# Okrio/tinyrecurrentunet

Measured on AMD Instinct MI355X. Metric: 16 kHz frames/sec (train step), higher is better.
Workload: dtype f32; 1 GPU; config/tiny.json TRU-Net (C_in=4 incl. PCEN), 64 x 4 s 16 kHz pairs per GPU, n_fft 512 hop 128, full fp32 train step; mfma=fp32 forward, bf16x3 backward, fp32_mfma=bf16x3-bwd, frames_per_gpu=32064, global_batch=64, parallelism=dp1

## Files before the change

tinyrecurrentunet_amd/csrc/dma_common.hpp:

```cpp
#pragma once
#include "common.hpp"

namespace {

typedef __attribute__((address_space(3))) void* lds_ptr_t;

#define VMCNT_0_31_(W_)                                                                                                \
    W_(0) W_(1) W_(2) W_(3) W_(4) W_(5) W_(6) W_(7) W_(8) W_(9) W_(10) W_(11) W_(12) W_(13) W_(14) W_(15)             \
    W_(16) W_(17) W_(18) W_(19) W_(20) W_(21) W_(22) W_(23) W_(24) W_(25) W_(26) W_(27) W_(28) W_(29) W_(30) W_(31)
#define VMCNT_32_60_(W_)                                                                                               \
    W_(32) W_(33) W_(34) W_(35) W_(36) W_(37) W_(38) W_(39) W_(40) W_(41) W_(42) W_(43) W_(44) W_(45) W_(46) W_(47)   \
    W_(48) W_(49) W_(50) W_(51) W_(52) W_(53) W_(54) W_(55) W_(56) W_(57) W_(58) W_(59) W_(60)
#define VMCNT_CASE_(k) case k: asm volatile("s_waitcnt vmcnt(" #k ")" ::: "memory"); break;
template <int MAXN>
__device__ __forceinline__ void wait_vmcnt_exact(int n) {
    static_assert(MAXN == 31 || MAXN == 60, "ranges with a case list");
    if constexpr (MAXN == 31) {
        switch (n) {
            VMCNT_0_31_(VMCNT_CASE_)
            default: asm volatile("s_waitcnt vmcnt(0)" ::: "memory"); break;
        }
    } else {
        switch (n) {
            VMCNT_0_31_(VMCNT_CASE_) VMCNT_32_60_(VMCNT_CASE_)
            default: asm volatile("s_waitcnt vmcnt(0)" ::: "memory"); break;
        }
    }
}
#undef VMCNT_CASE_
#undef VMCNT_32_60_
#undef VMCNT_0_31_

__device__ __forceinline__ int swz_off(int r, int pc) { return r * 32 + 4 * (pc ^ ((r >> 1) & 7)); }

__device__ __forceinline__ __amdgpu_buffer_rsrc_t buffer_rsrc(const void* base) {
    return __builtin_amdgcn_make_buffer_rsrc(const_cast<void*>(base), 0, 0x7fffffff, 0x00020000);
}

__device__ __forceinline__ int wave_uniform(int v) { return __builtin_amdgcn_readfirstlane(v); }

}
```

tinyrecurrentunet_amd/csrc/gemm_common.hpp:

```cpp
#pragma once
#include "dma_common.hpp"

namespace {


constexpr int NT = TRUNET_TILE_FRAMES;

template <int CT>
struct BVec;
template <>
struct BVec<4> { typedef f32x4 type; };
template <>
struct BVec<2> { typedef f32x2 type; };
template <>
struct BVec<1> { typedef float type; };

template <int CT>
__device__ __forceinline__ float vget(const typename BVec<CT>::type& v, int i) {
    if constexpr (CT == 1) return v; else return v[i];
}
template <int CT>
__device__ __forceinline__ void vset(typename BVec<CT>::type& v, int i, float x) {
    if constexpr (CT == 1) v = x; else v[i] = x;
}

struct SegPos { bool valid; int q; };

__device__ __forceinline__ SegPos seg_pos(const trunet_seg& sg, int p) {
    int qn = p * sg.pos_mul + sg.pos_off;
    SegPos r;
    const int sh = sg.pos_div >> 1;
    r.q = qn >> sh;
    r.valid = (qn >= 0) && ((qn & sh) == 0) && (r.q < sg.L);
    return r;
}

struct ChunkIt {
    int tile, tile_end, p, n0, s, cc, ach, cbase;
    bool valid;
    bool placed;
};

template <int KC, int FT = NT>
__device__ __forceinline__ void it_enter_tile(const trunet_gemm_args& a, ChunkIt& it) {
    it.valid = it.tile < it.tile_end;
    if (!it.valid) return;
    if (!it.placed) {
        const int nt = it.tile / a.P;
        it.p = a.p_begin + (it.tile - nt * a.P);
        it.n0 = nt * FT;
        it.placed = true;
    }
    it.s = 0; it.cc = 0; it.ach = 0; it.cbase = 0;
#ifdef GEMM_SIMPLE_IT
    return;
#endif
    while (it.s < a.nseg - 1 && !seg_pos(a.seg[it.s], it.p).valid) {
        it.ach += (a.seg[it.s].nchan + KC - 1) / KC;
        it.cbase += a.seg[it.s].nchan;
        ++it.s;
    }
}

template <int KC, int FT = NT>
__device__ __forceinline__ bool it_next(const trunet_gemm_args& a, ChunkIt& it) {
#ifdef GEMM_SIMPLE_IT
    if (++it.cc < (a.seg[0].nchan + KC - 1) / KC) return false;
    it.cc = 0;
    ++it.tile;
    if (++it.p == a.p_begin + a.P) { it.p = a.p_begin; it.n0 += FT; }
    it.valid = it.tile < it.tile_end;
    return true;
#endif
    const int nck = (a.seg[it.s].nchan + KC - 1) / KC;
    if (++it.cc < nck) return false;
    it.ach += nck;
    it.cbase += a.seg[it.s].nchan;
    it.cc = 0;
    ++it.s;
    while (it.s < a.nseg && !seg_pos(a.seg[it.s], it.p).valid) {
        it.ach += (a.seg[it.s].nchan + KC - 1) / KC;
        it.cbase += a.seg[it.s].nchan;
        ++it.s;
    }
    if (it.s < a.nseg) return false;
    ++it.tile;
    if (++it.p == a.p_begin + a.P) { it.p = a.p_begin; it.n0 += FT; }
    it_enter_tile<KC, FT>(a, it);
    return true;
}

__device__ __forceinline__ void wait_vmcnt(int n) {
    switch (n >> 2) {
        case 0: asm volatile("s_waitcnt vmcnt(0)" ::: "memory"); break;
        case 1: asm volatile("s_waitcnt vmcnt(4)" ::: "memory"); break;
        case 2: asm volatile("s_waitcnt vmcnt(8)" ::: "memory"); break;
        case 3: asm volatile("s_waitcnt vmcnt(12)" ::: "memory"); break;
        case 4: asm volatile("s_waitcnt vmcnt(16)" ::: "memory"); break;
        case 5: asm volatile("s_waitcnt vmcnt(20)" ::: "memory"); break;
        case 6: asm volatile("s_waitcnt vmcnt(24)" ::: "memory"); break;
        case 7: asm volatile("s_waitcnt vmcnt(28)" ::: "memory"); break;
        case 8: asm volatile("s_waitcnt vmcnt(32)" ::: "memory"); break;
        case 9: asm volatile("s_waitcnt vmcnt(36)" ::: "memory"); break;
        case 10: asm volatile("s_waitcnt vmcnt(40)" ::: "memory"); break;
        case 11: asm volatile("s_waitcnt vmcnt(44)" ::: "memory"); break;
        default: asm volatile("s_waitcnt vmcnt(48)" ::: "memory"); break;
    }
}

}
```

tinyrecurrentunet_amd/csrc/gemm_conv.hip:

```cpp
#include <cstdlib>
#include "common.hpp"

#include "gemm_common.hpp"

namespace {


template <int RS, int KC, bool TWO, int EPL, int NW>
__global__ __launch_bounds__(64 * NW, (EPL == 0 || NW == 8) ? 2 : 1) void conv_gemm_kernel(const trunet_gemm_args a, const int NB) {
    constexpr int FT = 32 * NW;
    constexpr int CT = RS;
    constexpr int CG = 4 / RS;
    constexpr int MB = 32 * RS;
    constexpr int KP = KC / 2;
    constexpr int NSRC = TWO ? 2 : 1;
    constexpr int CHF = KC * FT * NSRC;
    constexpr int LPW = (KC / 8) * NSRC;
    typedef typename BVec<CT>::type bvec;
    extern __shared__ __attribute__((aligned(16))) float smem[];

    const int tid = threadIdx.x;
    const int lane = tid & 63;
    const int wave8 = __builtin_amdgcn_readfirstlane(tid >> 6);
    const int half = wave8 >> 2;
    const int wave = wave8 & 3;
    const int rs = wave % RS;
    const int cg = wave / RS;
    const int h = lane >> 5;
    const int c = lane & 31;
    const int mblk = blockIdx.y;

    int nck_total = 0, nchan_total = 0;
    for (int s = 0; s < a.nseg; ++s) {
        nck_total += (a.seg[s].nchan + KC - 1) / KC;
        nchan_total += a.seg[s].nchan;
    }
    float* A_lds = smem;
    float* R_lds = A_lds + (size_t)nck_total * RS * (KP * 64);
    f32x4* C_lds = (f32x4*)(R_lds + (size_t)NB * CHF);
    float* E_lds = (float*)(C_lds + nchan_total);

    const int ntn = a.NP / FT;
    const int total_tiles = a.P * ntn;
    ChunkIt cur;
    cur.placed = false;
    cur.tile = (int)(((long long)blockIdx.x * total_tiles) / gridDim.x);
    cur.tile_end = (int)(((long long)(blockIdx.x + 1) * total_tiles) / gridDim.x);
    const bool has_work = cur.tile < cur.tile_end;

    float st1[16], st2[16];
#pragma unroll
    for (int r = 0; r < 16; ++r) { st1[r] = 0.f; st2[r] = 0.f; }

    if (has_work) {
        const int totalA = nck_total * RS * (KP * 64);
        for (int idx = tid; idx < totalA; idx += 64 * NW) {
            const int j = idx & 3;
            const int ln = (idx >> 2) & 63;
            const int rest = idx >> 8;
            const int kg = rest % (KP / 4);
            const int rest2 = rest / (KP / 4);
            const int rr = rest2 % RS;
            const int ch = rest2 / RS;
            int s = 0, cc = ch;
            while (cc >= (a.seg[s].nchan + KC - 1) / KC) { cc -= (a.seg[s].nchan + KC - 1) / KC; ++s; }
            const int kk = 4 * kg + j;
            const int ci = cc * KC + 2 * kk + (ln >> 5);
            const int m = mblk * MB + 32 * rr + (ln & 31);
            const bool ok = ci < a.seg[s].nchan && m < a.M;
            const float v = a.W[(size_t)(min(m, a.M - 1) + a.w_m_off) * a.ldw_m +
                                (size_t)min(ci, a.seg[s].nchan - 1) * a.ldw_c + a.seg[s].woff];
            A_lds[idx] = ok ? v : 0.f;
        }
        int base = 0;
        for (int s = 0; s < a.nseg; ++s) {
            const trunet_seg& sg = a.seg[s];
            for (int ci = tid; ci < sg.nchan; ci += 64 * NW) {
                f32x4 k;
                if (TWO) {
                    const bool on = sg.mode == TRUNET_PRO_BNBWD;
                    k[0] = on ? sg.c0[ci] : 1.f; k[1] = on ? sg.c1[ci] : 0.f; k[2] = on ? sg.c2[ci] : 0.f; k[3] = 0.f;
                } else {
                    const bool on = sg.mode == TRUNET_PRO_BNRELU;
                    k[0] = on ? sg.c0[ci] : 1.f; k[1] = on ? sg.c1[ci] : 0.f; k[2] = on ? 0.f : -3.0e38f; k[3] = 0.f;
                }
                C_lds[base + ci] = k;
            }
            base += sg.nchan;
        }
        for (int r = tid; r < MB; r += 64 * NW) {
            const int m = mblk * MB + r;
            const int mg = m + a.m_out_off;
            const bool ok = m < a.M;
            E_lds[r] = (ok && (a.epi & TRUNET_EPI_BIAS)) ? a.bias[mg] : 0.f;
            E_lds[MB + r] = (ok && EPL > 0) ? a.e0[mg] : 0.f;
            E_lds[2 * MB + r] = (ok && EPL > 0) ? a.e1[mg] : 0.f;
            E_lds[3 * MB + r] = (ok && EPL > 0 && a.e2) ? a.e2[mg] : 0.f;
        }
    }
    __syncthreads();

    if (has_work) {
        auto issue_dma = [&](const ChunkIt& it, int slot) {
            const trunet_seg& sg = a.seg[it.s];
            const int q = seg_pos(sg, it.p).q;
            float* dst = R_lds + (size_t)slot * CHF;
            const size_t boff = (size_t)q * a.NP + it.n0;
            const unsigned rstride = (unsigned)sg.L * (unsigned)a.NP;
            const float* b0 = sg.src0 + boff;
            const float* b1 = (TWO ? (sg.src1 ? sg.src1 : sg.src0) : sg.src0) + boff;
#pragma unroll
            for (int i = 0; i < LPW; ++i) {
                const int g = (LPW / NSRC) * wave8 + i / NSRC;
                const int e = g * 256 + 4 * lane;
                const int row = e / FT, col = e % FT;
                const int cch = min(it.cc * KC + row, sg.nchan - 1);
                const unsigned off = (unsigned)cch * rstride + (unsigned)col;
                const float* gp = ((TWO && (i % NSRC)) ? b1 : b0) + off;
                __builtin_amdgcn_global_load_lds(gp, (lds_ptr_t)(dst + (i % NSRC) * (KC * FT) + g * 256), 16, 0, TRUNET_DMA_AUX);
            }
        };
        auto transform = [&](const ChunkIt& it, int slot) {
            float* dst = R_lds + (size_t)slot * CHF;
            const int nrow = a.seg[it.s].nchan - it.cc * KC;
            f32x4 v[LPW / NSRC], z[LPW / NSRC], k[LPW / NSRC];
#pragma unroll
            for (int i = 0; i < LPW / NSRC; ++i) {
                const int e = ((LPW / NSRC) * wave8 + i) * 256 + 4 * lane;
                const float* pz = dst + e;
                v[i] = *(const f32x4*)pz;
                if (TWO) z[i] = *(const f32x4*)(pz + KC * FT);
                k[i] = C_lds[it.cbase + it.cc * KC + min(e / FT, nrow - 1)];
            }
#pragma unroll
            for (int i = 0; i < LPW / NSRC; ++i) {
                if (TWO) {
#pragma unroll
                    for (int e = 0; e < 4; ++e) v[i][e] = fmaf(k[i][0], v[i][e], fmaf(k[i][1], z[i][e], k[i][2]));
                } else {
#pragma unroll
                    for (int e = 0; e < 4; ++e) v[i][e] = fmaxf(fmaf(v[i][e], k[i][0], k[i][1]), k[i][2]);
                }
            }
#pragma unroll
            for (int i = 0; i < LPW / NSRC; ++i)
                *(f32x4*)(dst + ((LPW / NSRC) * wave8 + i) * 256 + 4 * lane) = v[i];
        };

        if (NW == 8 && wave8 >= 4) __builtin_amdgcn_s_setprio(1);
        it_enter_tile<KC, FT>(a, cur);
        ChunkIt ld = cur, ldlast = cur;
        for (int d = 0; d < NB; ++d) {
            if (ld.valid) ldlast = ld;
            issue_dma(ldlast, d);
            if (ld.valid) it_next<KC, FT>(a, ld);
        }
        ChunkIt tf = cur;
        int tslot = 0;
        wait_vmcnt((NB - 1) * LPW);
        transform(tf, tslot);
        it_next<KC, FT>(a, tf);
        tslot = 1;
        asm volatile("s_waitcnt lgkmcnt(0)" ::: "memory");
        __builtin_amdgcn_s_barrier();
        asm volatile("" ::: "memory");

        int slot = 0;
        while (cur.valid) {
            f32x16 acc[CT];
#pragma unroll
            for (int t = 0; t < CT; ++t)
#pragma unroll
                for (int r = 0; r < 16; ++r) acc[t][r] = 0.f;
            const int tp = cur.p;
            const int nb = cur.n0 + 128 * half + (32 * RS) * cg + CT * c;
            bvec zv[16], ov[16];
            bool last = false;
            while (!last) {
                ChunkIt nxt = cur;
                last = it_next<KC, FT>(a, nxt);
                if (EPL > 0 && last) {
#pragma unroll
                    for (int r = 0; r < 16; ++r) {
                        const int ml = 32 * rs + (r & 3) + 8 * (r >> 2) + 4 * h;
                        const int m = min(mblk * MB + ml, a.M - 1);
                        const size_t off = ((size_t)(m + a.m_out_off) * a.out_L + tp + a.out_pos_off) * a.NP + nb;
                        zv[r] = *(const bvec*)(a.zmask + off);
                        if (EPL > 1) ov[r] = *(const bvec*)(a.out + off);
                    }
                }
                if (tf.valid) {
                    if (EPL > 0 && last) asm volatile("s_waitcnt vmcnt(0)" ::: "memory");
                    else wait_vmcnt((NB - 2) * LPW);
                    transform(tf, tslot);
                    it_next<KC, FT>(a, tf);
                    tslot = (tslot + 1 == NB) ? 0 : tslot + 1;
                }
                {
                    const float* Ab = A_lds + (size_t)((cur.ach + cur.cc) * RS + rs) * (KP * 64);
                    const float* Bb = R_lds + (size_t)slot * CHF + 128 * half + (32 * RS) * cg + CT * c;
                    f32x4 af[KP / 4];
                    bvec bf[KP];
#pragma unroll
                    for (int kg = 0; kg < KP / 4; ++kg) af[kg] = *(const f32x4*)(Ab + (kg * 64 + lane) * 4);
#pragma unroll
                    for (int kk = 0; kk < KP; ++kk) bf[kk] = *(const bvec*)(Bb + (2 * kk + h) * FT);
#pragma unroll
                    for (int kk = 0; kk < KP; ++kk)
#pragma unroll
                        for (int t = 0; t < CT; ++t)
                            acc[t] = __builtin_amdgcn_mfma_f32_32x32x2f32(af[kk >> 2][kk & 3], vget<CT>(bf[kk], t),
                                                                          acc[t], 0, 0, 0);
                    constexpr int LA = 1 + 4 / CT;
                    __builtin_amdgcn_sched_group_barrier(0x100, KP / 4 + LA, 0);
#pragma unroll
                    for (int kk = 0; kk < KP - LA; ++kk) {
                        __builtin_amdgcn_sched_group_barrier(0x008, CT, 0);
                        __builtin_amdgcn_sched_group_barrier(0x100, 1, 0);
                    }
                    __builtin_amdgcn_sched_group_barrier(0x008, LA * CT, 0);
                }
                asm volatile("" ::: "memory");
                __builtin_amdgcn_s_barrier();
                asm volatile("" ::: "memory");
                if (ld.valid) ldlast = ld;
                issue_dma(ldlast, slot);
                if (ld.valid) it_next<KC, FT>(a, ld);
                slot = (slot + 1 == NB) ? 0 : slot + 1;
                cur = nxt;
            }
#pragma unroll
            for (int r = 0; r < 16; ++r) {
                const int ml = 32 * rs + (r & 3) + 8 * (r >> 2) + 4 * h;
                const int m = mblk * MB + ml;
                const int mg = m + a.m_out_off;
                const size_t off = ((size_t)mg * a.out_L + tp + a.out_pos_off) * a.NP + nb;
                bvec val;
                const float bv = E_lds[ml];
#pragma unroll
                for (int t = 0; t < CT; ++t) vset<CT>(val, t, acc[t][r] + bv);
                if (EPL > 1) {
#pragma unroll
                    for (int t = 0; t < CT; ++t) vset<CT>(val, t, vget<CT>(val, t) + vget<CT>(ov[r], t));
                }
                float e2 = 0.f;
                if (EPL > 0) {
                    const float e0 = E_lds[MB + ml], e1 = E_lds[2 * MB + ml];
                    e2 = E_lds[3 * MB + ml];
#pragma unroll
                    for (int t = 0; t < CT; ++t)
                        vset<CT>(val, t, (fmaf(e0, vget<CT>(zv[r], t), e1) > 0.f) ? vget<CT>(val, t) : 0.f);
                }
                if (a.epi & TRUNET_EPI_RELU) {
#pragma unroll
                    for (int t = 0; t < CT; ++t) vset<CT>(val, t, fmaxf(vget<CT>(val, t), 0.f));
                }
#ifdef TRUNET_EPI_NT
                if (m < a.M) __builtin_nontemporal_store(val, (bvec*)(a.out + off));
#else
                if (m < a.M) *(bvec*)(a.out + off) = val;
#endif
                if (a.epi & TRUNET_EPI_STATS) {
#pragma unroll
                    for (int t = 0; t < CT; ++t) {
                        const float x = (nb + t < a.N && m < a.M) ? vget<CT>(val, t) : 0.f;
                        st1[r] += x;
                        if (EPL > 0) st2[r] = fmaf(x, vget<CT>(zv[r], t) - e2, st2[r]);
                        else st2[r] = fmaf(x, x, st2[r]);
                    }
                }
            }
        }
        asm volatile("s_waitcnt vmcnt(0)" ::: "memory");
    }

    if (a.epi & TRUNET_EPI_STATS) {
#pragma unroll
        for (int r = 0; r < 16; ++r) {
            float s1 = half_wave_sum(st1[r]);
            float s2 = half_wave_sum(st2[r]);
            const int ml = (r & 3) + 8 * (r >> 2) + 4 * h;
            const int m = mblk * MB + 32 * rs + ml;
            if (c == 0 && m < a.M) {
                const int mg = m + a.m_out_off;
                float* pp = a.partials + ((size_t)((blockIdx.x * (NW / 4) + half) * CG + cg) * a.M_stat + mg) * 2;
                pp[0] = s1;
                pp[1] = s2;
            }
        }
    }
}


template <int EPL>
__global__ __launch_bounds__(256) void conv_smallm_kernel(const trunet_gemm_args a) {
    extern __shared__ __attribute__((aligned(16))) float smem[];
    __shared__ double red[256];
    int nchan_total = 0;
    for (int s = 0; s < a.nseg; ++s) nchan_total += a.seg[s].nchan;
    f32x4* Wl = (f32x4*)smem;
    f32x4* Cl = Wl + 2 * nchan_total;
    const int tid = threadIdx.x;
    {
        int base = 0;
        for (int s = 0; s < a.nseg; ++s) {
            const trunet_seg& sg = a.seg[s];
            for (int ci = tid; ci < sg.nchan; ci += 256) {
                float w[8];
#pragma unroll
                for (int m = 0; m < 8; ++m)
                    w[m] = (m < a.M) ? a.W[(size_t)(m + a.w_m_off) * a.ldw_m + (size_t)ci * a.ldw_c + sg.woff] : 0.f;
                f32x4 w0 = {w[0], w[1], w[2], w[3]}, w1 = {w[4], w[5], w[6], w[7]};
                Wl[2 * (base + ci)] = w0;
                Wl[2 * (base + ci) + 1] = w1;
                const bool on = sg.mode == TRUNET_PRO_BNRELU;
                f32x4 k = {on ? sg.c0[ci] : 1.f, on ? sg.c1[ci] : 0.f, on ? 0.f : -3.0e38f, 0.f};
                Cl[base + ci] = k;
            }
            base += sg.nchan;
        }
    }
    __syncthreads();
    const int f4 = tid & 63, py = tid >> 6;
    const int ntn = (a.NP + 255) / 256;
    const int items = a.P * ntn;
    float s1[8], s2[8];
#pragma unroll
    for (int m = 0; m < 8; ++m) { s1[m] = 0.f; s2[m] = 0.f; }
    for (int it = blockIdx.x * 4 + py; it < items; it += gridDim.x * 4) {
        const int nt = it / a.P;
        const int p = a.p_begin + (it - nt * a.P);
        const int n = nt * 256 + 4 * f4;
        if (n >= a.NP) continue;
        f32x4 acc[8];
#pragma unroll
        for (int m = 0; m < 8; ++m) acc[m] = f32x4{0.f, 0.f, 0.f, 0.f};
        int cb = 0;
        for (int s = 0; s < a.nseg; ++s) {
            const trunet_seg& sg = a.seg[s];
            const SegPos sp = seg_pos(sg, p);
            if (sp.valid) {
                const float* src = sg.src0 + (size_t)sp.q * a.NP + n;
                const size_t cstr = (size_t)sg.L * a.NP;
                for (int c0 = 0; c0 < sg.nchan; c0 += 8) {
                    f32x4 v[8];
#pragma unroll
                    for (int j = 0; j < 8; ++j) {
                        const int ci = min(c0 + j, sg.nchan - 1);
#ifdef TRUNET_THIN_NT
                        v[j] = __builtin_nontemporal_load((const f32x4*)(src + ci * cstr));
#else
                        v[j] = *(const f32x4*)(src + ci * cstr);
#endif
                    }
#pragma unroll
                    for (int j = 0; j < 8; ++j) {
                        const int ci = c0 + j;
                        if (ci < sg.nchan) {
                            const f32x4 k = Cl[cb + ci];
                            const f32x4 w0 = Wl[2 * (cb + ci)], w1 = Wl[2 * (cb + ci) + 1];
#pragma unroll
                            for (int e = 0; e < 4; ++e) v[j][e] = fmaxf(fmaf(v[j][e], k[0], k[1]), k[2]);
#pragma unroll
                            for (int m = 0; m < 4; ++m)
#pragma unroll
                                for (int e = 0; e < 4; ++e) {
                                    acc[m][e] = fmaf(w0[m], v[j][e], acc[m][e]);
                                    acc[4 + m][e] = fmaf(w1[m], v[j][e], acc[4 + m][e]);
                                }
                        }
                    }
                }
            }
            cb += sg.nchan;
        }
#pragma unroll
        for (int m = 0; m < 8; ++m) {
            if (m < a.M) {
                const int mg = m + a.m_out_off;
                const size_t off = ((size_t)mg * a.out_L + p + a.out_pos_off) * a.NP + n;
                f32x4 val = acc[m];
                if (a.epi & TRUNET_EPI_BIAS) {
                    const float bv = a.bias[mg];
#pragma unroll
                    for (int e = 0; e < 4; ++e) val[e] += bv;
                }
                f32x4 zv = {0.f, 0.f, 0.f, 0.f};
                float e2 = 0.f;
                if (EPL > 1) {
                    const f32x4 old = *(const f32x4*)(a.out + off);
#pragma unroll
                    for (int e = 0; e < 4; ++e) val[e] += old[e];
                }
                if (EPL > 0) {
                    zv = *(const f32x4*)(a.zmask + off);
                    const float e0 = a.e0[mg], e1 = a.e1[mg];
                    e2 = a.e2 ? a.e2[mg] : 0.f;
#pragma unroll
                    for (int e = 0; e < 4; ++e) val[e] = (fmaf(e0, zv[e], e1) > 0.f) ? val[e] : 0.f;
                }
                if (a.epi & TRUNET_EPI_RELU) {
#pragma unroll
                    for (int e = 0; e < 4; ++e) val[e] = fmaxf(val[e], 0.f);
                }
                *(f32x4*)(a.out + off) = val;
                if (a.epi & TRUNET_EPI_STATS) {
#pragma unroll
                    for (int e = 0; e < 4; ++e) {
                        const float x = (n + e < a.N) ? val[e] : 0.f;
                        s1[m] += x;
                        s2[m] = (EPL > 0) ? fmaf(x, zv[e] - e2, s2[m]) : fmaf(x, x, s2[m]);
                    }
                }
            }
        }
    }
    if (a.epi & TRUNET_EPI_STATS) {
#pragma unroll
        for (int m = 0; m < 8; ++m) {
            const double r1 = block_sum_f64((double)s1[m], red);
            const double r2 = block_sum_f64((double)s2[m], red);
            if (tid == 0 && m < a.M) {
                float* pp = a.partials + ((size_t)blockIdx.x * a.M_stat + m + a.m_out_off) * 2;
                pp[0] = (float)r1;
                pp[1] = (float)r2;
            }
        }
    }
}

int launch_smallm(const trunet_gemm_args* h, hipStream_t st) {
    int nchan_total = 0;
    for (int s = 0; s < h->nseg; ++s) nchan_total += h->seg[s].nchan;
    const size_t lds = (size_t)nchan_total * 3 * sizeof(f32x4);
    const int epl = (h->epi & TRUNET_EPI_MASK) ? ((h->epi & TRUNET_EPI_ACCUM) ? 2 : 1) : 0;
    const int items = h->P * ((h->NP + 255) / 256);
    int grid = (items + 3) / 4;
    if (grid > 1024) grid = 1024;
    if (epl == 0) hipLaunchKernelGGL(conv_smallm_kernel<0>, dim3(grid), dim3(256), lds, st, *h);
    else if (epl == 1) hipLaunchKernelGGL(conv_smallm_kernel<1>, dim3(grid), dim3(256), lds, st, *h);
    else hipLaunchKernelGGL(conv_smallm_kernel<2>, dim3(grid), dim3(256), lds, st, *h);
    return trunet_launch_status();
}

template <int RS, int KC, bool TWO, int EPL, int NW>
int launch_gemm_nw(const trunet_gemm_args* h, int NB, size_t lds, hipStream_t st) {
    const int mb = 32 * RS;
    dim3 grid((NW == 4 && EPL == 0 && lds <= 80 * 1024) ? 2 * TRUNET_NUM_CU : TRUNET_NUM_CU, (h->M + mb - 1) / mb);
    auto kern = conv_gemm_kernel<RS, KC, TWO, EPL, NW>;
    if (hipFuncSetAttribute((const void*)kern, hipFuncAttributeMaxDynamicSharedMemorySize, (int)lds) != hipSuccess)
        return TRUNET_ELAUNCH;
    hipLaunchKernelGGL(kern, grid, dim3(64 * NW), lds, st, *h, NB);
    return trunet_launch_status();
}

template <int RS, int KC, bool TWO, int EPL>
int launch_gemm(const trunet_gemm_args* h, int NB, size_t lds, hipStream_t st, int nw = 4) {
    if constexpr (EPL == 0 || (EPL == 1 && RS <= 2)) {
        if (nw == 8) return launch_gemm_nw<RS, KC, TWO, EPL, 8>(h, NB, lds, st);
    }
    return launch_gemm_nw<RS, KC, TWO, EPL, 4>(h, NB, lds, st);
}

template <int RS>
int launch_gemm_rs(const trunet_gemm_args* h, int kc, bool two, int epl, int NB, size_t lds, hipStream_t st, int nw) {
    if constexpr (RS == 2) {
        if (two && kc == 8) {
            if (epl == 0) return launch_gemm<RS, 8, true, 0>(h, NB, lds, st, nw);
            if (epl == 1) return launch_gemm<RS, 8, true, 1>(h, NB, lds, st, nw);
            return launch_gemm<RS, 8, true, 2>(h, NB, lds, st, nw);
        }
    }
    if (two && kc == 32) {
        if (epl == 0) return launch_gemm<RS, 32, true, 0>(h, NB, lds, st, nw);
        if (epl == 1) return launch_gemm<RS, 32, true, 1>(h, NB, lds, st, nw);
        return launch_gemm<RS, 32, true, 2>(h, NB, lds, st, nw);
    }
    if (two) {
        if (epl == 0) return launch_gemm<RS, 16, true, 0>(h, NB, lds, st, nw);
        if (epl == 1) return launch_gemm<RS, 16, true, 1>(h, NB, lds, st, nw);
        return launch_gemm<RS, 16, true, 2>(h, NB, lds, st, nw);
    }
    if (epl == 0) return launch_gemm<RS, 32, false, 0>(h, NB, lds, st, nw);
    if (epl == 1) return launch_gemm<RS, 32, false, 1>(h, NB, lds, st, nw);
    return launch_gemm<RS, 32, false, 2>(h, NB, lds, st, nw);
}

struct GemmPlan { int rs, kc, nb, nw; size_t lds; bool two; int epl; };

int plan_gemm(const trunet_gemm_args* h, GemmPlan* pl) {
    bool two = false;
    int nchan_total = 0, kpad32 = 0;
    for (int s = 0; s < h->nseg; ++s) {
        two = two || h->seg[s].mode == TRUNET_PRO_BNBWD;
        nchan_total += h->seg[s].nchan;
        kpad32 += (h->seg[s].nchan + 31) / 32 * 32;
    }
    int rs0 = h->M > 64 ? 4 : (h->M > 32 ? 2 : 1);
    const size_t budget = 160 * 1024;
    static const bool kc8_ok = !(getenv("TRUNET_GEMM_KC8") && getenv("TRUNET_GEMM_KC8")[0] == '0');
    const bool thin_k = kc8_ok && two && rs0 == 2 && h->nseg == 1 && nchan_total <= 8;
    for (int rs = rs0; rs >= 1; rs >>= 1) {
        for (int kc = thin_k ? 8 : 32; kc >= (thin_k ? 8 : (two ? 16 : 32)); kc >>= 1) {
            int kpad = 0;
            for (int s = 0; s < h->nseg; ++s) kpad += (h->seg[s].nchan + kc - 1) / kc * kc;
            const size_t slot = (size_t)kc * NT * sizeof(float) * (two ? 2 : 1);
            const size_t fixed = (size_t)kpad * rs * 128 + (size_t)nchan_total * 16 + 4 * 32 * rs * sizeof(float);
            if (fixed + 3 * slot > budget) continue;
            int nb = (int)((budget - fixed) / slot);
            if (nb > 6) nb = 6;
            if (!(h->epi & TRUNET_EPI_MASK) && fixed + 2 * slot <= budget / 2) nb = (int)((budget / 2 - fixed) / slot);
            pl->rs = rs; pl->kc = kc; pl->nb = nb; pl->lds = fixed + nb * slot; pl->two = two; pl->nw = 4;
            static const bool wide_ok = !(getenv("TRUNET_GEMM_WIDE") && getenv("TRUNET_GEMM_WIDE")[0] == '0');
            const int epl_w = (h->epi & TRUNET_EPI_MASK) ? ((h->epi & TRUNET_EPI_ACCUM) ? 2 : 1) : 0;
            const bool wide_kind = epl_w == 0 || (epl_w == 1 && rs <= 2);
            if (wide_ok && wide_kind && (h->NP % 256) == 0 && fixed + 2 * 2 * slot <= budget &&
                (pl->lds > 80 * 1024 || epl_w > 0)) {
                int nbw = (int)((budget - fixed) / (2 * slot));
                if (nbw > 4) nbw = 4;
                pl->nw = 8; pl->nb = nbw; pl->lds = fixed + (size_t)nbw * 2 * slot;
            } else if (wide_ok && wide_kind && two && kc == 32 && (h->NP % 256) == 0) {
                int kpad16 = 0;
                for (int s = 0; s < h->nseg; ++s) kpad16 += (h->seg[s].nchan + 15) / 16 * 16;
                const size_t slot16 = (size_t)16 * NT * sizeof(float) * 2;
                const size_t fixed16 = (size_t)kpad16 * rs * 128 + (size_t)nchan_total * 16 + 4 * 32 * rs * sizeof(float);
                if (fixed16 + 2 * 2 * slot16 <= budget) {
                    int nbw = (int)((budget - fixed16) / (2 * slot16));
                    if (nbw > 4) nbw = 4;
                    pl->kc = 16; pl->nw = 8; pl->nb = nbw; pl->lds = fixed16 + (size_t)nbw * 2 * slot16;
                }
            }
            pl->epl = (h->epi & TRUNET_EPI_MASK) ? ((h->epi & TRUNET_EPI_ACCUM) ? 2 : 1) : 0;
            return TRUNET_OK;
        }
    }
    (void)kpad32;
    return TRUNET_ENOTSUP;
}

}

int trunet_gemm_x3_plan(const trunet_gemm_args* h, int* nb, size_t* lds);
int trunet_launch_gemm_x3(const trunet_gemm_args* h, int nrt, int nb, size_t lds, hipStream_t st);

extern "C" int trunet_conv_gemm_plan(const trunet_gemm_args* h, int* rs, int* kc, int* nb, int* two, int* epl, int* nw) {
    if (!h || !rs || !kc || !nb || !two || !epl || !nw) return TRUNET_EINVAL;
    {
        int xnb = 0;
        size_t xlds = 0;
        const int nrt = (h->M > 8) ? trunet_gemm_x3_plan(h, &xnb, &xlds) : 0;
        if (nrt) {
            *rs = nrt; *kc = 16; *nb = xnb; *two = 0; *epl = 0; *nw = -8;
            return TRUNET_OK;
        }
    }
    GemmPlan pl;
    if (plan_gemm(h, &pl) != TRUNET_OK) return TRUNET_ENOTSUP;
    *rs = pl.rs; *kc = pl.kc; *nb = pl.nb; *two = pl.two ? 1 : 0; *epl = pl.epl; *nw = pl.nw;
    return TRUNET_OK;
}

extern "C" int trunet_conv_gemm_nparts(int M) {
    (void)M;
    return TRUNET_NUM_CU * 8;
}

extern "C" int trunet_conv_gemm(const trunet_gemm_args* h, void* stream) {
    if (!h || !h->out || !h->W || h->nseg < 1 || h->nseg > TRUNET_MAX_SEG) return TRUNET_EINVAL;
    if (h->NP <= 0 || (h->NP % NT) != 0 || h->N > h->NP || h->P <= 0 || h->M <= 0) return TRUNET_EINVAL;
    if ((h->epi & TRUNET_EPI_STATS) && !h->partials) return TRUNET_EINVAL;
    if ((h->epi & TRUNET_EPI_MASK) && (!h->zmask || !h->e0 || !h->e1)) return TRUNET_EINVAL;
    if ((h->epi & TRUNET_EPI_ACCUM) && !(h->epi & TRUNET_EPI_MASK)) return TRUNET_ENOTSUP;
    if ((h->epi & TRUNET_EPI_BIAS) && !h->bias) return TRUNET_EINVAL;
    if (h->out_L <= 0 || h->p_begin < 0 || h->m_out_off < 0 || h->p_begin + h->out_pos_off < 0 ||
        h->p_begin + h->P + h->out_pos_off > h->out_L)
        return TRUNET_EINVAL;
    if ((h->epi & TRUNET_EPI_STATS) && h->M_stat < h->M + h->m_out_off) return TRUNET_EINVAL;
    bool any_two = false, any_relu = false;
    for (int s = 0; s < h->nseg; ++s) {
        const trunet_seg& sg = h->seg[s];
        if (!sg.src0 || sg.nchan <= 0 || sg.pos_div <= 0 || sg.L <= 0) return TRUNET_EINVAL;
        if (sg.pos_div > 2) return TRUNET_ENOTSUP;
        if (sg.mode == TRUNET_PRO_BNBWD && (!sg.src1 || !sg.c0 || !sg.c1 || !sg.c2)) return TRUNET_EINVAL;
        if (sg.mode == TRUNET_PRO_BNRELU && (!sg.c0 || !sg.c1)) return TRUNET_EINVAL;
        any_two = any_two || sg.mode == TRUNET_PRO_BNBWD;
        any_relu = any_relu || sg.mode == TRUNET_PRO_BNRELU;
    }
    if (any_two && any_relu) return TRUNET_ENOTSUP;
    GemmPlan pl;
    if (plan_gemm(h, &pl) != TRUNET_OK) return TRUNET_ENOTSUP;
    hipStream_t st = (hipStream_t)stream;
    if ((h->epi & TRUNET_EPI_STATS) && !(h->epi & TRUNET_EPI_PREZERO)) {
        size_t bytes = (size_t)trunet_conv_gemm_nparts(h->M) * h->M_stat * 2 * sizeof(float);
        if (hipMemsetAsync(h->partials, 0, bytes, st) != hipSuccess) return TRUNET_ELAUNCH;
    }
    if (h->M <= 8 && !any_two) return launch_smallm(h, st);
    {
        int xnb = 0;
        size_t xlds = 0;
        const int nrt = trunet_gemm_x3_plan(h, &xnb, &xlds);
        if (nrt) return trunet_launch_gemm_x3(h, nrt, xnb, xlds, st);
    }
    switch (pl.rs) {
        case 4: return launch_gemm_rs<4>(h, pl.kc, pl.two, pl.epl, pl.nb, pl.lds, st, pl.nw);
        case 2: return launch_gemm_rs<2>(h, pl.kc, pl.two, pl.epl, pl.nb, pl.lds, st, pl.nw);
        default: return launch_gemm_rs<1>(h, pl.kc, pl.two, pl.epl, pl.nb, pl.lds, st, pl.nw);
// ... 405 lines not shown
```

tinyrecurrentunet_amd/engine.py:

```python
import torch

from . import _lib as L
import os

from ._lib import (DG_ACCUM, DG_MASK, DG_PREZERO, DG_STATS, DG_STORE, EPI_ACCUM, EPI_BIAS, EPI_MASK, EPI_PREZERO, EPI_STATS, PRO_BNBWD,
                   PRO_BNRELU, PRO_NONE, ConvtBwdArgs, GemmArgs, PwBwdArgs, WgradArgs, check, make_seg, ptr)

F_BINS = 257
FRAME_PAD = 256
BN_EPS = 1e-5
BN_MOM = 0.1


FUSED_PWBWD = os.environ.get("TRUNET_FUSED_PWBWD", "1") != "0"
DW_RZ = os.environ.get("TRUNET_DW_RZ", "1") != "0"

FUSED_THIN = os.environ.get("TRUNET_FUSED_THIN", "1") != "0"
FUSED_GRU_PROJ = os.environ.get("TRUNET_FUSED_GRU_PROJ", "1") != "0"

FUSED_CONVT = os.environ.get("TRUNET_FUSED_CONVT", "1") != "0"

TGRU_LOOP = os.environ.get("TRUNET_TGRU_LOOP", "0") == "1"

PROFILE = None
PROFILE_LOG = None
PROFILE_BYTES = {}


class _Timed:
    def __init__(self, name, flops=0.0, tag="", nbytes=0.0):
        self.name, self.flops, self.tag, self.nbytes = name, flops, tag, nbytes

    def __enter__(self):
        if PROFILE is not None:
            self.a = torch.cuda.Event(enable_timing=True)
            self.b = torch.cuda.Event(enable_timing=True)
            self.a.record()
        return self

    def __exit__(self, *exc):
        if PROFILE is not None:
            self.b.record()
            PROFILE.setdefault(self.name, []).append((self.a, self.b, self.flops))
            if self.nbytes:
                PROFILE_BYTES[self.name] = PROFILE_BYTES.get(self.name, 0.0) + self.nbytes
            if PROFILE_LOG is not None:
                PROFILE_LOG.append((self.name, self.tag, self.a, self.b, self.flops))
        return False


def _gemm_rs(M, segs):
    nck = sum((s.nchan + 31) // 32 for s in segs)
    rs = 4 if M > 64 else (2 if M > 32 else 1)
    while rs > 1 and nck * rs * 4096 > 112 * 1024:
        rs >>= 1
    return rs


def _gemm_kernel_name(a):
    import ctypes as C
    v = [C.c_int() for _ in range(6)]
    check(L.lib().trunet_conv_gemm_plan(a, *[C.byref(x) for x in v]), "conv_gemm_plan")
    rs, kc, nb, two, epl, nw = [x.value for x in v]
    if a.M <= 8 and not two:
        return "conv_smallm_kernel<%d>" % epl
    if nw < 0:
        return "conv_gemm_x3_kernel<%d>" % rs
    return "conv_gemm_kernel<%d, %d, %s, %d, %d>" % (rs, kc, "true" if two else "false", epl, nw)


def _seg_positions(s, p0, P):
    n = 0
    for p in range(p0, p0 + P):
        qn = p * s.pos_mul + s.pos_off
        if qn >= 0 and qn % s.pos_div == 0 and qn // s.pos_div < s.L:
            n += 1
    return n


def ceil_to(n, m):
    return (n + m - 1) // m * m


class BNState:

    def __init__(self, C, dev):
        z = lambda: torch.empty(C, device=dev, dtype=torch.float32)
        self.C = C
        self.scale, self.shift, self.mean, self.rstd = z(), z(), z(), z()
        self.ca, self.cb, self.cc = z(), z(), z()
        self.count = 0.0
        self.module = None


class Act:

    def __init__(self, t, C, Ln, bn=None):
        self.t, self.C, self.L, self.bn = t, C, Ln, bn

    def seg(self, pos_off=0, woff=0, pos_mul=1, pos_div=1):
        if self.bn is None:
            return make_seg(self.t, self.C, self.L, pos_mul, pos_off, pos_div, woff, PRO_NONE)
        return make_seg(self.t, self.C, self.L, pos_mul, pos_off, pos_div, woff, PRO_BNRELU,
                        c0=self.bn.scale, c1=self.bn.shift)


class Workspace:

    def __init__(self, dev):
        self.dev = dev
        self.t = {}
        self.gen = 0
        self.pending = set()

    def take_clean(self, name):
        clean = name not in self.pending
        self.pending.add(name)
        return clean

    def get(self, name, shape, zero=False, dtype=torch.float32):
        t = self.t.get(name)
        if t is None or tuple(t.shape) != tuple(shape) or t.dtype != dtype:
            t = (torch.zeros if zero else torch.empty)(shape, device=self.dev, dtype=dtype)
            self.t[name] = t
        elif zero:
            t.zero_()
        return t

    def flat(self, name, numel, zero=False, dtype=torch.float32):
        t = self.t.get(name)
        if t is None or t.numel() < numel:
            t = (torch.zeros if zero else torch.empty)(max(numel, 1), device=self.dev, dtype=dtype)
            self.t[name] = t
            self.pending.discard(name)
        return t

    def zero_crop(self, t, q0, q1):
        key = "crop0:%d" % id(t)
        if self.t.get(key) is not None and self.t[key][0] is t and self.t[key][1:] == (q0, q1):
            return
        if q0 > 0:
            t[:, :q0].zero_()
        if q1 < t.shape[1]:
            t[:, q1:].zero_()
        self.t[key] = (t, q0, q1)

    def bn(self, name, C):
        b = self.t.get("bn:" + name)
        if b is None:
            b = BNState(C, self.dev)
            self.t["bn:" + name] = b
        return b


class TRUNetEngine:
    ENC = [(3, 1), (5, 2), (3, 1), (5, 2), (3, 2)]
    DEC = [(3, 2), (5, 2), (3, 1), (5, 2), (3, 1), (5, 2)]

    def __init__(self, net):
        self.net = net
        self._ws = {}

    def ws(self, NP, dev, record=False):
        key = (NP, str(dev), bool(record))
        if key not in self._ws:
            self._ws = {k: v for k, v in self._ws.items() if k[2] != key[2]}
            self._ws[key] = Workspace(dev)
        return self._ws[key]

    @staticmethod
    def _check_gen(w, gen):
        if w.gen != gen:
            raise L.TrunetHipError(
                "backward() of a forward whose saved activations were overwritten: another gradient-recording forward of "
                "the same module ran before this backward (forward #%d, workspace is at #%d).  Call backward() before "
                "the next training forward (no_grad / eval forwards in between are fine)." % (gen, w.gen))

    def _gemm(self, w, *, N, NP, P, M, out, out_L, W, ldw_m, ldw_c, segs, p_begin=0, out_pos_off=0, m_out_off=0,
              w_m_off=0, epi=0, bias=None, zmask=None, e0=None, e1=None, e2=None, stats=None):
        a = GemmArgs()
        a.NP, a.N, a.P, a.p_begin = NP, N, P, p_begin
        a.M, a.m_out_off, a.out_L, a.out_pos_off = M, m_out_off, out_L, out_pos_off
        a.ldw_m, a.ldw_c, a.w_m_off = ldw_m, ldw_c, w_m_off
        a.nseg = len(segs)
        for i, s in enumerate(segs):
            a.seg[i] = s
        a.out, a.W = ptr(out), ptr(W)
        if bias is not None:
            epi |= EPI_BIAS
            a.bias = ptr(bias)
        if zmask is not None:
            epi |= EPI_MASK
            a.zmask, a.e0, a.e1, a.e2 = ptr(zmask), ptr(e0), ptr(e1), ptr(e2)
        nparts = 0
        if stats is not None:
            epi |= EPI_STATS
            nparts = L.lib().trunet_conv_gemm_nparts(M)
            part = w.flat("partials", nparts * stats * 2, zero=True)
            a.partials, a.M_stat = ptr(part), stats
            if w.take_clean("partials"):
                epi |= EPI_PREZERO
        a.epi = epi
        if PROFILE is not None:
            fl = 2.0 * N * M * sum(s.nchan * _seg_positions(s, p_begin, P) for s in segs)
            tag = "M%d K%s P%d%s%s" % (M, "+".join(str(s.nchan) for s in segs), P,
                                       " two" if any(s.mode == PRO_BNBWD for s in segs) else "",
                                       " mask" if zmask is not None else "")
            with _Timed(_gemm_kernel_name(a), fl, tag):
                check(L.lib().trunet_conv_gemm(a, L.stream()), "conv_gemm")
            return nparts
        check(L.lib().trunet_conv_gemm(a, L.stream()), "conv_gemm")
        return nparts

    def _gemm_args(self, *, N, NP, P, M, out, out_L, W, ldw_m, ldw_c, segs, bias=None, p_begin=0):
        a = GemmArgs()
        a.NP, a.N, a.P, a.p_begin = NP, N, P, p_begin
        a.M, a.m_out_off, a.out_L, a.out_pos_off = M, 0, out_L, 0
        a.ldw_m, a.ldw_c, a.w_m_off = ldw_m, ldw_c, 0
        a.nseg = len(segs)
        for i, sg in enumerate(segs):
            a.seg[i] = sg
# ... 789 lines not shown
```

Measured before the change: 757,900 frames/s.

## Add fast buffer-store epilogue and compile-time pipeline depth to conv GEMM

```diff
diff --git a/tinyrecurrentunet_amd/csrc/dma_common.hpp b/tinyrecurrentunet_amd/csrc/dma_common.hpp
--- a/tinyrecurrentunet_amd/csrc/dma_common.hpp
+++ b/tinyrecurrentunet_amd/csrc/dma_common.hpp
@@ -39,4 +39,28 @@
 
 __device__ __forceinline__ int wave_uniform(int v) { return __builtin_amdgcn_readfirstlane(v); }
 
+template <typename T>
+__device__ __forceinline__ T* wave_uniform_ptr(T* p) {
+    const unsigned long long v = (unsigned long long)p;
+    const unsigned lo = (unsigned)__builtin_amdgcn_readfirstlane((int)(unsigned)v);
+    const unsigned hi = (unsigned)__builtin_amdgcn_readfirstlane((int)(unsigned)(v >> 32));
+    return (T*)(((unsigned long long)hi << 32) | lo);
 }
+
+typedef unsigned u32x2 __attribute__((ext_vector_type(2)));
+typedef unsigned u32x4 __attribute__((ext_vector_type(4)));
+__device__ __forceinline__ void buffer_store_row(__amdgpu_buffer_rsrc_t r, int voff, int soff, float v) {
+    __builtin_amdgcn_raw_buffer_store_b32(__builtin_bit_cast(unsigned, v), r, voff, soff, 0);
+}
+__device__ __forceinline__ void buffer_store_row(__amdgpu_buffer_rsrc_t r, int voff, int soff, f32x2 v) {
+    __builtin_amdgcn_raw_buffer_store_b64(__builtin_bit_cast(u32x2, v), r, voff, soff, 0);
+}
+__device__ __forceinline__ void buffer_store_row(__amdgpu_buffer_rsrc_t r, int voff, int soff, f32x4 v) {
+    __builtin_amdgcn_raw_buffer_store_b128(__builtin_bit_cast(u32x4, v), r, voff, soff, 0);
+}
+__device__ __forceinline__ float keep_scalar(float x) {
+    asm("" : "+v"(x));
+    return x;
+}
+
+}
diff --git a/tinyrecurrentunet_amd/csrc/gemm_common.hpp b/tinyrecurrentunet_amd/csrc/gemm_common.hpp
--- a/tinyrecurrentunet_amd/csrc/gemm_common.hpp
+++ b/tinyrecurrentunet_amd/csrc/gemm_common.hpp
@@ -23,6 +23,8 @@
 __device__ __forceinline__ void vset(typename BVec<CT>::type& v, int i, float x) {
     if constexpr (CT == 1) v = x; else v[i] = x;
 }
+
+__host__ __device__ constexpr int frag_row(int r) { return (r & 3) + 8 * (r >> 2); }
 
 struct SegPos { bool valid; int q; };
 
diff --git a/tinyrecurrentunet_amd/csrc/gemm_conv.hip b/tinyrecurrentunet_amd/csrc/gemm_conv.hip
--- a/tinyrecurrentunet_amd/csrc/gemm_conv.hip
+++ b/tinyrecurrentunet_amd/csrc/gemm_conv.hip
@@ -1,4 +1,5 @@
 #include <cstdlib>
+#include <type_traits>
 #include "common.hpp"
 
 #include "gemm_common.hpp"
@@ -6,8 +7,10 @@
 namespace {
 
 
-template <int RS, int KC, bool TWO, int EPL, int NW>
-__global__ __launch_bounds__(64 * NW, (EPL == 0 || NW == 8) ? 2 : 1) void conv_gemm_kernel(const trunet_gemm_args a, const int NB) {
+template <int RS, int KC, bool TWO, int EPL, int NW, int NBT>
+__global__ __launch_bounds__(64 * NW, (EPL == 0 || NW == 8) ? 2 : 1) void conv_gemm_kernel(const trunet_gemm_args a, const int nb_rt,
+                                                                                          const int buf_rows) {
+    const int NB = NBT ? NBT : nb_rt;
     constexpr int FT = 32 * NW;
     constexpr int CT = RS;
     constexpr int CG = 4 / RS;
@@ -148,6 +151,25 @@
         };
 
         if (NW == 8 && wave8 >= 4) __builtin_amdgcn_s_setprio(1);
+        constexpr bool PREG = EPL == 0;
+        float bvr[PREG ? 16 : 1];
+        if (PREG) {
+#pragma unroll
+            for (int r = 0; r < 16; ++r) bvr[r] = E_lds[32 * rs + frag_row(r) + 4 * h];
+        }
+        const bool relu = (a.epi & TRUNET_EPI_RELU) != 0;
+        const bool stats = (a.epi & TRUNET_EPI_STATS) != 0;
+#ifdef TRUNET_EPI_NT
+        const bool fast = false;
+#else
+        const bool fast = EPL == 0 && buf_rows && !relu && mblk * MB + MB <= a.M;
+#endif
+        const size_t rowstride = (size_t)a.out_L * a.NP;
+        int voffq[4];
+#pragma unroll
+        for (int q = 0; q < 4; ++q) voffq[q] = fast ? (int)(((4 * h + q) * rowstride + CT * c) * sizeof(float)) : 0;
+        const size_t row0 = (size_t)(mblk * MB + 32 * rs + a.m_out_off) * a.out_L + a.out_pos_off;
+        const int wcol = 128 * half + (32 * RS) * cg;
         it_enter_tile<KC, FT>(a, cur);
         ChunkIt ld = cur, ldlast = cur;
         for (int d = 0; d < NB; ++d) {
@@ -173,7 +195,9 @@
 #pragma unroll
                 for (int r = 0; r < 16; ++r) acc[t][r] = 0.f;
             const int tp = cur.p;
-            const int nb = cur.n0 + 128 * half + (32 * RS) * cg + CT * c;
+            const int tn0 = cur.n0;
+            const int nb = tn0 + wcol + CT * c;
+            const size_t tbase = (row0 + tp) * a.NP + tn0 + wcol;
             bvec zv[16], ov[16];
             bool last = false;
             while (!last) {
@@ -182,7 +206,7 @@
                 if (EPL > 0 && last) {
 #pragma unroll
                     for (int r = 0; r < 16; ++r) {
-                        const int ml = 32 * rs + (r & 3) + 8 * (r >> 2) + 4 * h;
+                        const int ml = 32 * rs + frag_row(r) + 4 * h;
                         const int m = min(mblk * MB + ml, a.M - 1);
                         const size_t off = ((size_t)(m + a.m_out_off) * a.out_L + tp + a.out_pos_off) * a.NP + nb;
                         zv[r] = *(const bvec*)(a.zmask + off);
@@ -229,44 +253,70 @@
                 slot = (slot + 1 == NB) ? 0 : slot + 1;
                 cur = nxt;
             }
-#pragma unroll
-            for (int r = 0; r < 16; ++r) {
-                const int ml = 32 * rs + (r & 3) + 8 * (r >> 2) + 4 * h;
-                const int m = mblk * MB + ml;
-                const int mg = m + a.m_out_off;
-                const size_t off = ((size_t)mg * a.out_L + tp + a.out_pos_off) * a.NP + nb;
-                bvec val;
-                const float bv = E_lds[ml];
-#pragma unroll
-                for (int t = 0; t < CT; ++t) vset<CT>(val, t, acc[t][r] + bv);
-                if (EPL > 1) {
-#pragma unroll
-                    for (int t = 0; t < CT; ++t) vset<CT>(val, t, vget<CT>(val, t) + vget<CT>(ov[r], t));
-                }
-                float e2 = 0.f;
-                if (EPL > 0) {
-                    const float e0 = E_lds[MB + ml], e1 = E_lds[2 * MB + ml];
-                    e2 = E_lds[3 * MB + ml];
-#pragma unroll
-                    for (int t = 0; t < CT; ++t)
-                        vset<CT>(val, t, (fmaf(e0, vget<CT>(zv[r], t), e1) > 0.f) ? vget<CT>(val, t) : 0.f);
-                }
-                if (a.epi & TRUNET_EPI_RELU) {
-#pragma unroll
-                    for (int t = 0; t < CT; ++t) vset<CT>(val, t, fmaxf(vget<CT>(val, t), 0.f));
-                }
+            if (fast) {
+                __amdgpu_buffer_rsrc_t ro[4];
+#pragma unroll
+                for (int g = 0; g < 4; ++g) ro[g] = buffer_rsrc(wave_uniform_ptr(a.out + tbase + 8 * g * rowstride));
+                auto rows = [&](auto with_stats, auto partial) {
+#pragma unroll
+                    for (int r = 0; r < 16; ++r) {
+                        bvec val;
+#pragma unroll
+                        for (int t = 0; t < CT; ++t) vset<CT>(val, t, keep_scalar(acc[t][r] + bvr[PREG ? r : 0]));
+                        buffer_store_row(ro[r >> 2], voffq[r & 3], 0, val);
+                        if (decltype(with_stats)::value) {
+#pragma unroll
+                            for (int t = 0; t < CT; ++t) {
+                                const float x = (decltype(partial)::value && nb + t >= a.N) ? 0.f : vget<CT>(val, t);
+                                st1[r] = keep_scalar(st1[r] + x);
+                                st2[r] = keep_scalar(fmaf(x, x, st2[r]));
+                            }
+                        }
+                    }
+                };
+                if (!stats) rows(std::false_type(), std::false_type());
+                else if (tn0 + FT > a.N) rows(std::true_type(), std::true_type());
+                else rows(std::true_type(), std::false_type());
+            } else {
+#pragma unroll
+                for (int r = 0; r < 16; ++r) {
+                    const int ml = 32 * rs + frag_row(r) + 4 * h;
+                    const int m = mblk * MB + ml;
+                    const int mg = m + a.m_out_off;
+                    const size_t off = ((size_t)mg * a.out_L + tp + a.out_pos_off) * a.NP + nb;
+                    bvec val;
+                    const float bv = PREG ? bvr[PREG ? r : 0] : E_lds[ml];
+#pragma unroll
+                    for (int t = 0; t < CT; ++t) vset<CT>(val, t, acc[t][r] + bv);
+                    if (EPL > 1) {
+#pragma unroll
+                        for (int t = 0; t < CT; ++t) vset<CT>(val, t, vget<CT>(val, t) + vget<CT>(ov[r], t));
+                    }
+                    float e2 = 0.f;
+                    if (EPL > 0) {
+                        const float e0 = E_lds[MB + ml], e1 = E_lds[2 * MB + ml];
+                        e2 = E_lds[3 * MB + ml];
+#pragma unroll
+                        for (int t = 0; t < CT; ++t)
+                            vset<CT>(val, t, (fmaf(e0, vget<CT>(zv[r], t), e1) > 0.f) ? vget<CT>(val, t) : 0.f);
+                    }
+                    if (relu) {
+#pragma unroll
+                        for (int t = 0; t < CT; ++t) vset<CT>(val, t, fmaxf(vget<CT>(val, t), 0.f));
+                    }
 #ifdef TRUNET_EPI_NT
-                if (m < a.M) __builtin_nontemporal_store(val, (bvec*)(a.out + off));
+                    if (m < a.M) __builtin_nontemporal_store(val, (bvec*)(a.out + off));
 #else
-                if (m < a.M) *(bvec*)(a.out + off) = val;
+                    if (m < a.M) *(bvec*)(a.out + off) = val;
 #endif
-                if (a.epi & TRUNET_EPI_STATS) {
-#pragma unroll
-                    for (int t = 0; t < CT; ++t) {
-                        const float x = (nb + t < a.N && m < a.M) ? vget<CT>(val, t) : 0.f;
-                        st1[r] += x;
-                        if (EPL > 0) st2[r] = fmaf(x, vget<CT>(zv[r], t) - e2, st2[r]);
-                        else st2[r] = fmaf(x, x, st2[r]);
+                    if (stats) {
+#pragma unroll
+                        for (int t = 0; t < CT; ++t) {
+                            const float x = (nb + t < a.N && m < a.M) ? vget<CT>(val, t) : 0.f;
+                            st1[r] += x;
+                            if (EPL > 0) st2[r] = fmaf(x, vget<CT>(zv[r], t) - e2, st2[r]);
+                            else st2[r] = fmaf(x, x, st2[r]);
+                        }
                     }
                 }
             }
@@ -443,15 +493,26 @@
     return trunet_launch_status();
 }
 
+template <int RS, int KC, bool TWO, int EPL, int NW, int NBT>
+int launch_gemm_nb(const trunet_gemm_args* h, int NB, size_t lds, hipStream_t st) {
+    const int mb = 32 * RS;
+    dim3 grid((NW == 4 && EPL == 0 && lds <= 80 * 1024) ? 2 * TRUNET_NUM_CU : TRUNET_NUM_CU, (h->M + mb - 1) / mb);
+    auto kern = conv_gemm_kernel<RS, KC, TWO, EPL, NW, NBT>;
+    if (hipFuncSetAttribute((const void*)kern, hipFuncAttributeMaxDynamicSharedMemorySize, (int)lds) != hipSuccess)
+        return TRUNET_ELAUNCH;
+    const long long span = 32LL * h->out_L * h->NP * (long long)sizeof(float) + 32 * NW * (long long)sizeof(float);
+    const int buf_rows = span < (1LL << 31) ? 1 : 0;
+    hipLaunchKernelGGL(kern, grid, dim3(64 * NW), lds, st, *h, NB, buf_rows);
+    return trunet_launch_status();
+}
+
 template <int RS, int KC, bool TWO, int EPL, int NW>
 int launch_gemm_nw(const trunet_gemm_args* h, int NB, size_t lds, hipStream_t st) {
-    const int mb = 32 * RS;
-    dim3 grid((NW == 4 && EPL == 0 && lds <= 80 * 1024) ? 2 * TRUNET_NUM_CU : TRUNET_NUM_CU, (h->M + mb - 1) / mb);
-    auto kern = conv_gemm_kernel<RS, KC, TWO, EPL, NW>;
-    if (hipFuncSetAttribute((const void*)kern, hipFuncAttributeMaxDynamicSharedMemorySize, (int)lds) != hipSuccess)
-        return TRUNET_ELAUNCH;
-    hipLaunchKernelGGL(kern, grid, dim3(64 * NW), lds, st, *h, NB);
-    return trunet_launch_status();
+    if constexpr (!TWO && EPL == 0 && RS >= 2) {
+        if (NB == 2) return launch_gemm_nb<RS, KC, TWO, EPL, NW, 2>(h, NB, lds, st);
+        if (NB == 3) return launch_gemm_nb<RS, KC, TWO, EPL, NW, 3>(h, NB, lds, st);
+    }
+    return launch_gemm_nb<RS, KC, TWO, EPL, NW, 0>(h, NB, lds, st);
 }
 
 template <int RS, int KC, bool TWO, int EPL>
diff --git a/tinyrecurrentunet_amd/engine.py b/tinyrecurrentunet_amd/engine.py
--- a/tinyrecurrentunet_amd/engine.py
+++ b/tinyrecurrentunet_amd/engine.py
@@ -66,7 +66,8 @@
         return "conv_smallm_kernel<%d>" % epl
     if nw < 0:
         return "conv_gemm_x3_kernel<%d>" % rs
-    return "conv_gemm_kernel<%d, %d, %s, %d, %d>" % (rs, kc, "true" if two else "false", epl, nw)
+    nbt = nb if (not two and epl == 0 and rs >= 2 and nb in (2, 3)) else 0
+    return "conv_gemm_kernel<%d, %d, %s, %d, %d, %d>" % (rs, kc, "true" if two else "false", epl, nw, nbt)
 
 
 def _seg_positions(s, p0, P):
```

After: 766,500 frames/s, median of 6. +1.1%, better.
